# beecave-homelab/VibeVoice-ROCm

Measured on AMD Instinct MI355X. Metric: audio-sec/s, higher is better.
Workload: dtype bf16; 1 GPU; cfg2: VibeVoice-1.5B shapes, 1 speaker(s) x 203-frame voice prompt, 330-token prompt, 225 frames (30.0 s audio), CFG=2.0, 20 DPM-Solver++ steps, whole generate() incl. voice encode + prefill; global_batch=1, parallelism=replicas x1 (one dialogue per GPU), hipgraph=True

## Files before the change

vibevoice_rocm_amd/csrc/vv_common.h:

```cpp
#ifndef VV_COMMON_H
#define VV_COMMON_H
#include <hip/hip_runtime.h>
#include <stdarg.h>
#include <stdint.h>
#include "vv_hip.h"

int vv_set_error(int code, const char* fmt, ...);

#define VV_CHECK_LAUNCH(name)                                                                    \
  do {                                                                                           \
    hipError_t e_ = hipGetLastError();                                                           \
    if (e_ != hipSuccess) return vv_set_error(VV_E_HIP, "%s: %s", name, hipGetErrorString(e_));  \
  } while (0)

#define VV_TRY(expr)            \
  do {                          \
    int rc_ = (expr);           \
    if (rc_) return rc_;        \
  } while (0)

int vv_launch_gemv_stream(const vv_lin_args& a, hipStream_t s);
int vv_launch_gemv_rows(const vv_lin_args& a, float* part, size_t part_floats, int* tickets, size_t n_tickets, hipStream_t s);
size_t vv_gemv_rows_part_floats(int n, int dual);
size_t vv_gemv_rows_tickets(int n);
int vv_gemv_rows_init();
void vv_gemv_rows_set(int on, int blocks, int pers);
int vv_linear_ws(const vv_lin_args* a, const void* f1, const void* f2, float* part, size_t part_floats, int* tickets, size_t n_tickets,
                 vv_stream_t stream, const vv_w8* q1 = nullptr, const vv_w8* q2 = nullptr);
int vv_launch_mfma_gemm(const vv_lin_args& a, hipStream_t s);
int vv_mfma_gemm_init();
int vv_launch_attn_decode(const float* qkv, int64_t ld_qkv, int R, int heads, const vv_kv* kv, int layer, const float2* rope, const int* lens, float* out,
                          int64_t ldo, float* part, int* tickets, int nsplit, int part_cap, hipStream_t s);
int vv_attn_decode_ws(const float* qkv, int64_t ld_qkv, int R, int heads, const vv_kv* kv, int layer, const float* rope_table, const int* lens, float* out,
                      int64_t ldo, float* part, int* tickets, int nsplit, int part_cap, vv_stream_t stream);
int vv_launch_attn_prefill(const float* qkv, int64_t ld_qkv, int R, int heads, const vv_kv* kv, int layer, const int* lens, const int* cache_rows,
                           float* out, int64_t ldo, hipStream_t s);
int vv_head_init_fused(const vv_head* h, const float* noise, float* Xs, float* Ms, float* h0, int64_t ldh, hipStream_t s);
bool vv_head_boundary_supported(const vv_head* h);
int vv_head_boundary_fused(const vv_head* h, const float* hrows, int64_t ldh, const float* shift, const float* scale, int64_t ld_mod, float cfg,
                           const vv_dpm_coef* k, float* Xs, float* Ms, float* h_out, int64_t ldh_out, float* latent_out, hipStream_t s);
int vv_head_boundary_batch(const vv_head* h, const float* hrows, int64_t ldh, const float* shift, const float* scale, int64_t ld_mod, float cfg,
                           const vv_dpm_coef* k, float* Xs, float* Ms, int64_t state_stride, float* h_out, int64_t ldh_out, float* latent_out,
                           int64_t latent_stride, int B, hipStream_t s,
                           const float* nx = nullptr, int64_t nx_stride = 0);
int vv_head_sde_proj_fused(const vv_head* h, const float* sde_noise, int64_t ld_sde, int n_steps, int B, float* NX, hipStream_t s);
int vv_fused_init();
int vv_head_pre_fused(const vv_head* h, const float* cond2, int64_t ld_cond, const float* temb, int n_steps, void* c_bf16, const float* noise,
                      float* Xs, float* Ms, float* h0, int64_t ldh, hipStream_t s);
int vv_launch_connector_pair(const vv_connector* ac, const vv_connector* sem, const float* latent, const float* semfeat, float* out, int64_t ldo, int rows_out,
                             float* ws, hipStream_t s);
int vv_head_modulations_fused(const vv_head* h, const void* c_bf16, int rows, float* const* mod, float* modf, hipStream_t s);
struct vv_conv_ctx_item { float* pad; float* state; int ctx, T, C; const float* dw_w; float* hs; int affine; float scale, bias; };
int vv_conv_ctx_batch(const vv_conv_ctx_item* items, int n, int scatter, hipStream_t s);
int vv_block1d_init();
int vv_launch_block1d(const vv_block& B, int wdt, const float* x, float* out, int T, int C, float eps, hipStream_t s);
void vv_block1d_set_fused(int on);
void vv_block1d_set_blocks(int b);
int vv_convffn_init();
int vv_launch_convffn(const vv_block& B, int wdt, const float* x, float* y, void* hidden, float* hist_new, float* out, int T, int C, float eps,
                      hipStream_t s);
void vv_convffn_set(int on);
int vv_launch_ffn_in_row(const vv_block& B, int wdt, const float* x, float* y, float* hidden, float* hist_new, int C, float eps, hipStream_t s);
void vv_convffn_set_t1(int on);
int vv_launch_ffn_in_row_hs(const vv_block& B, int wdt, const float* x, float* y, float* hidden, float* hist_new, int C, float eps, hipStream_t s);
void vv_convffn_set_t1hs(int on);
void vv_convffn_set_rows(int c, int rows);
void vv_convffn_set_c128(int on);
bool vv_convffn_prefers(int wdt, int T, int C);
int vv_launch_skinny(const vv_lin_args& a, hipStream_t s);
void vv_skinny_set(int on, int min_m, int max_m);
int vv_rmsnorm_rows(const float* x, int64_t ldx, const float* w, float eps, int rows, int n, float* out, int64_t ldo, hipStream_t s);

#ifdef __HIPCC__
__device__ __forceinline__ float vv_gelu_as(float v) {
  const float x = v * 0.70710678118654752440f, ax = fabsf(x);
  const float t = __builtin_amdgcn_rcpf(fmaf(0.3275911f, ax, 1.0f));
  const float poly = t * fmaf(t, fmaf(t, fmaf(t, fmaf(t, 1.061405429f, -1.453152027f), 1.421413741f), -0.284496736f), 0.254829592f);
  const float erf_abs = 1.0f - poly * __expf(-ax * ax);
  return 0.5f * v * (1.0f + copysignf(erf_abs, x));
}

__device__ __forceinline__ float vv_wave_sum(float v) {
#define VV_DPP_ADD(ctrl) v += __int_as_float(__builtin_amdgcn_update_dpp(0, __float_as_int(v), ctrl, 0xF, 0xF, true))
  VV_DPP_ADD(0xB1);
  VV_DPP_ADD(0x4E);
  VV_DPP_ADD(0x141);
  VV_DPP_ADD(0x140);
#undef VV_DPP_ADD
  const float r0 = __int_as_float(__builtin_amdgcn_readlane(__float_as_int(v), 0));
  const float r1 = __int_as_float(__builtin_amdgcn_readlane(__float_as_int(v), 16));
  const float r2 = __int_as_float(__builtin_amdgcn_readlane(__float_as_int(v), 32));
  const float r3 = __int_as_float(__builtin_amdgcn_readlane(__float_as_int(v), 48));
  return (r0 + r1) + (r2 + r3);
}
#endif

#endif
```

vibevoice_rocm_amd/csrc/vv_convffn.hip:

```cpp
#include <hip/hip_runtime.h>
#include <hip/hip_bf16.h>
#include <stdint.h>

#include "vv_hip.h"
#include "vv_common.h"

namespace {

typedef unsigned short bf16_t;
typedef __bf16 bf16x8 __attribute__((ext_vector_type(8)));
typedef float f32x16 __attribute__((ext_vector_type(16)));
typedef float f32x4 __attribute__((ext_vector_type(4)));
typedef unsigned int u32x4 __attribute__((ext_vector_type(4)));

#ifdef VV_CF_TIMING
__device__ unsigned long long g_cf_t[8];
#define CSTAMP(i) do { if (blockIdx.x == 0 && blockIdx.y == 0 && threadIdx.x == 0) { const long long t_ = wall_clock64(); g_cf_t[i] += (unsigned long long)(t_ - tprev_); tprev_ = t_; } } while (0)
#else
#define CSTAMP(i) do { } while (0)
#endif

constexpr int TR2 = 16;
constexpr int HALO = 6;

__device__ __forceinline__ unsigned int pack2(float a, float b) {
  const __hip_bfloat16 x = __float2bfloat16(a), y = __float2bfloat16(b);
  return (unsigned int)(*reinterpret_cast<const bf16_t*>(&x)) | ((unsigned int)(*reinterpret_cast<const bf16_t*>(&y)) << 16);
}
__device__ __forceinline__ float sq4(const float4 v) { return v.x * v.x + v.y * v.y + v.z * v.z + v.w * v.w; }

template <int C, int TRV, int NT = 256> struct InLay {
  static constexpr int VW = C >= 256 ? 4 : 2;
  static constexpr int F4 = C / 4;
  static constexpr int FV = C / VW;
  static constexpr int TPR = FV < NT ? FV : NT;
  static constexpr int NWV = NT / 64;
  static constexpr int CPT = FV / TPR;
  static constexpr int RP = NT / TPR;
  static constexpr int NI = (TRV + HALO + RP - 1) / RP;
  static constexpr int WR = NI * RP;
  static constexpr int WPR = TPR / 64;
  static constexpr int P1 = C + 8;
  static constexpr int ST = C / (16 * NWV);
  static constexpr size_t XN = (size_t)WR * C * 4;
  static constexpr size_t RED = (size_t)NWV * 16 * 64 * 4;
  static constexpr size_t XH = (size_t)(WR - HALO) * P1 * 2;
  static constexpr size_t PART = (size_t)2 * WR * 8 * 4;
  static constexpr size_t LDS = (XN > RED ? XN : RED) + XH + PART;
};

template <int VW> __device__ __forceinline__ void ldv(const float* p, float (&o)[VW]) {
  if constexpr (VW == 4) { const float4 t = *reinterpret_cast<const float4*>(p); o[0] = t.x; o[1] = t.y; o[2] = t.z; o[3] = t.w; }
  else { const float2 t = *reinterpret_cast<const float2*>(p); o[0] = t.x; o[1] = t.y; }
}
template <int VW> __device__ __forceinline__ void stv(float* p, const float (&o)[VW]) {
  if constexpr (VW == 4) *reinterpret_cast<float4*>(p) = make_float4(o[0], o[1], o[2], o[3]);
  else *reinterpret_cast<float2*>(p) = make_float2(o[0], o[1]);
}

template <int C, int TRV, bool HF32, int NT>
__global__ __launch_bounds__(NT) void ffn_in_kernel(const float* __restrict__ x, float* __restrict__ y, void* __restrict__ hidden_v,
                                                     float* __restrict__ hist_new, int T, const vv_block B, float eps) {
  using L = InLay<C, TRV, NT>;
  constexpr int TR = TRV, CPT = L::CPT, VW = L::VW, NWV = L::NWV;
#ifdef VV_CF_TIMING
  long long tprev_ = wall_clock64();
#endif
  extern __shared__ __attribute__((aligned(16))) unsigned char smem[];
  float* xn = reinterpret_cast<float*>(smem);
  float* red = reinterpret_cast<float*>(smem);
  bf16_t* xh = reinterpret_cast<bf16_t*>(smem + (L::XN > L::RED ? L::XN : L::RED));
  float* part = reinterpret_cast<float*>(smem + (L::XN > L::RED ? L::XN : L::RED) + L::XH);
  float* part2 = part + L::WR * 8;
  const int tid = threadIdx.x, lane = tid & 63, wave = __builtin_amdgcn_readfirstlane(tid >> 6);
  const int n0 = blockIdx.x * 32;
  const int t0 = blockIdx.y * TR;
  const int rows = min(TR, T - t0);
  const int lm = lane & 31, hk = (lane >> 5) * 8;

  const int rloc = wave / L::WPR, slot = wave % L::WPR;
  int c0[CPT];
#pragma unroll
  for (int j = 0; j < CPT; ++j) c0[j] = VW * (tid % L::TPR + L::TPR * j);
  const float* hb = B.hist ? B.hist : x;
  const float hkeep = B.hist ? 1.f : 0.f;
  float own[L::NI][CPT][VW];
#pragma unroll
  for (int i = 0; i < L::NI; ++i) {
    const int w = rloc + L::RP * i, t = t0 - HALO + w;
    const bool isx = t >= 0;
    const float* src = isx ? x + (int64_t)min(t, T - 1) * C : hb + (int64_t)(B.hist ? HALO + t : 0) * C;
    const float keep = (w < rows + HALO) ? (isx ? 1.f : hkeep) : 0.f;
#pragma unroll
    for (int j = 0; j < CPT; ++j) {
      ldv<VW>(src + c0[j], own[i][j]);
#pragma unroll
      for (int e = 0; e < VW; ++e) own[i][j][e] *= keep;
    }
  }
  float nw[CPT][VW], db[CPT][VW], gm[CPT][VW], fw[CPT][VW];
  float tap[CPT][VW * 7];
#pragma unroll
  for (int j = 0; j < CPT; ++j) {
    ldv<VW>(B.norm_w + c0[j], nw[j]);
    ldv<VW>(B.dw_b + c0[j], db[j]);
    ldv<VW>(B.gamma + c0[j], gm[j]);
    ldv<VW>(B.ffn_norm_w + c0[j], fw[j]);
#pragma unroll
    for (int q = 0; q < 7; ++q) {
      float tq[VW];
      ldv<VW>(B.dw_w + (size_t)c0[j] * 7 + VW * q, tq);
#pragma unroll
      for (int e = 0; e < VW; ++e) tap[j][VW * q + e] = tq[e];
    }
  }
// ... 29 lines not shown
    for (int sl = 1; sl < L::WPR; ++sl) ss += part[w * 8 + sl];
    const bool isx = t >= 0;
    const float rstd = isx ? rsqrtf(ss / (float)C + eps) : 1.f;
#pragma unroll
    for (int j = 0; j < CPT; ++j) {
      float o[VW];
#pragma unroll
      for (int e = 0; e < VW; ++e) o[e] = own[i][j][e] * rstd * (isx ? nw[j][e] : 1.f);
      stv<VW>(xn + w * C + c0[j], o);
    }
  }
  __syncthreads();
  CSTAMP(2);

  float y1[L::NI][CPT][VW];
#pragma unroll
  for (int i = 0; i < L::NI; ++i) {
#pragma unroll
    for (int j = 0; j < CPT; ++j)
#pragma unroll
      for (int e = 0; e < VW; ++e) y1[i][j][e] = 0.f;
    if (L::RP * i + L::RP - 1 < HALO) continue;
    const int w = rloc + L::RP * i, tt = w - HALO;
    const int tc = max(tt, 0);
    const float ok = (tt >= 0 && tt < rows) ? 1.f : 0.f;
    float q = 0.f;
#pragma unroll
    for (int j = 0; j < CPT; ++j) {
      float s[VW];
#pragma unroll
      for (int e = 0; e < VW; ++e) s[e] = db[j][e];
#pragma unroll
      for (int k = 0; k < 7; ++k) {
        float v[VW];
        ldv<VW>(xn + (tc + k) * C + c0[j], v);
#pragma unroll
        for (int e = 0; e < VW; ++e) s[e] = fmaf(tap[j][7 * e + k], v[e], s[e]);
      }
#pragma unroll
      for (int e = 0; e < VW; ++e) {
        y1[i][j][e] = (own[i][j][e] + gm[j][e] * s[e]) * ok;
        q = fmaf(y1[i][j][e], y1[i][j][e], q);
      }
    }
    const float s2 = vv_wave_sum(q);
    if (lane == 0) part2[w * 8 + slot] = s2;
  }
  if (hist_new && blockIdx.x == 0 && t0 + TR >= T) {
    for (int e = tid; e < HALO * L::F4; e += NT) {
      const int j = e / L::F4, c4 = e - j * L::F4;
      *reinterpret_cast<float4*>(hist_new + (size_t)j * C + 4 * c4) = *reinterpret_cast<const float4*>(xn + (size_t)(T - t0 + j) * C + 4 * c4);
    }
  }
  __syncthreads();
  CSTAMP(3);
  {
    const int ys0 = blockIdx.x * (C / (int)gridDim.x);
#pragma unroll
    for (int i = 0; i < L::NI; ++i) {
      if (L::RP * i + L::RP - 1 < HALO) continue;
      const int w = rloc + L::RP * i, tt = w - HALO;
      if (tt >= 0) {
        float ss = part2[w * 8];
#pragma unroll
        for (int sl = 1; sl < L::WPR; ++sl) ss += part2[w * 8 + sl];
        const float rstd = rsqrtf(ss / (float)C + eps);
#pragma unroll
        for (int j = 0; j < CPT; ++j) {
          if constexpr (VW == 4) {
            uint2 p;
            p.x = pack2(y1[i][j][0] * rstd * fw[j][0], y1[i][j][1] * rstd * fw[j][1]);
            p.y = pack2(y1[i][j][2] * rstd * fw[j][2], y1[i][j][3] * rstd * fw[j][3]);
            *reinterpret_cast<uint2*>(xh + tt * L::P1 + c0[j]) = p;
          } else {
            *reinterpret_cast<unsigned int*>(xh + tt * L::P1 + c0[j]) = pack2(y1[i][j][0] * rstd * fw[j][0], y1[i][j][1] * rstd * fw[j][1]);
          }
          const bool mine = c0[j] >= ys0 && c0[j] < ys0 + C / (int)gridDim.x;
          if (mine && tt < rows) stv<VW>(y + (int64_t)(t0 + tt) * C + c0[j], y1[i][j]);
        }
      }
    }
  }
  __syncthreads();

  CSTAMP(4);
  f32x16 acc;
#pragma unroll
  for (int i = 0; i < 16; ++i) acc[i] = 0.f;
  {
    const bf16_t* xf = xh + min(lm, TR - 1) * L::P1 + wave * (C / NWV) + hk;
#pragma unroll
    for (int s = 0; s < L::ST; ++s) {
      const u32x4 xb = *reinterpret_cast<const u32x4*>(xf + s * 16);
      acc = __builtin_amdgcn_mfma_f32_32x32x16_bf16(__builtin_bit_cast(bf16x8, wf[s]), __builtin_bit_cast(bf16x8, xb), acc, 0, 0, 0);
    }
  }
#pragma unroll
  for (int r = 0; r < 16; ++r) red[(wave * 16 + r) * 64 + lane] = acc[r];
  __syncthreads();
  CSTAMP(5);
  {
    const int m = lane & 31;
    if (m < rows && wave < 4) {
      float v[4];
#pragma unroll
      for (int i = 0; i < 4; ++i) {
// ... 79 lines not shown
    }
  q2 = vv_wave_sum(q2);
  if (lane == 0) part[4 + wave] = q2;
  if (keeper) {
#pragma unroll
    for (int j = 0; j < 2; ++j) {
#pragma unroll
      for (int r = 0; r < 5; ++r) stv<4>(hist_new + (size_t)r * C + c0[j], hrow[r][j]);
      stv<4>(hist_new + (size_t)5 * C + c0[j], xn[j]);
    }
  }
  __syncthreads();
  const float rstd2 = rsqrtf(((part[4] + part[5]) + (part[6] + part[7])) / (float)C + eps);
  {
    const int ys0 = blockIdx.x * (C / (int)gridDim.x);
#pragma unroll
    for (int j = 0; j < 2; ++j) {
      uint2 p;
      p.x = pack2(yv[j][0] * rstd2 * fw[j][0], yv[j][1] * rstd2 * fw[j][1]);
      p.y = pack2(yv[j][2] * rstd2 * fw[j][2], yv[j][3] * rstd2 * fw[j][3]);
      *reinterpret_cast<uint2*>(xh + c0[j]) = p;
      if (c0[j] >= ys0 && c0[j] < ys0 + C / (int)gridDim.x) stv<4>(y + c0[j], yv[j]);
    }
  }
  __syncthreads();
  f32x16 acc;
#pragma unroll
  for (int i = 0; i < 16; ++i) acc[i] = 0.f;
  {
    const bf16_t* xf = xh + wave * (C / 4) + hk;
#pragma unroll
    for (int s = 0; s < ST; ++s) {
      const u32x4 xb = *reinterpret_cast<const u32x4*>(xf + s * 16);
      acc = __builtin_amdgcn_mfma_f32_32x32x16_bf16(__builtin_bit_cast(bf16x8, wf[s]), __builtin_bit_cast(bf16x8, xb), acc, 0, 0, 0);
    }
  }
#pragma unroll
  for (int r = 0; r < 16; ++r) red[(wave * 16 + r) * 64 + lane] = acc[r];
  __syncthreads();
  if ((lane & 31) == 0) {
    float v[4];
#pragma unroll
    for (int i = 0; i < 4; ++i) {
      float s = 0.f;
#pragma unroll
      for (int w4 = 0; w4 < 4; ++w4) s += red[(w4 * 16 + 4 * eg + i) * 64 + lane];
      v[i] = s;
    }
    *reinterpret_cast<float4*>(hidden + n0 + 8 * eg + 4 * (lane >> 5)) =
        make_float4(vv_gelu_as(v[0] + b1v.x), vv_gelu_as(v[1] + b1v.y), vv_gelu_as(v[2] + b1v.z), vv_gelu_as(v[3] + b1v.w));
  }
}

template <int C, int NW>
__global__ __launch_bounds__(64 * NW) void ffn_out_kernel(const bf16_t* __restrict__ hidden, const float* res, float* out, const float* __restrict__ hist_new,
                                                          int T, const vv_block B) {
  constexpr int K = 4 * C, KW = K / NW, ST = KW / 32;
  __shared__ float red[NW * 4 * 64];
  const int tid = threadIdx.x, lane = tid & 63, wave = tid >> 6;
  const int n0 = blockIdx.x * 16, t0 = blockIdx.y * TR2;
  const int r16 = lane & 15, kq = lane >> 4;
  u32x4 wf[ST], hf[ST];
  {
    const bf16_t* wr = reinterpret_cast<const bf16_t*>(B.w2) + (int64_t)(n0 + r16) * K + wave * KW + 8 * kq;
    const bf16_t* hr = hidden + (int64_t)min(t0 + r16, T - 1) * K + wave * KW + 8 * kq;
#pragma unroll
    for (int s = 0; s < ST; ++s) {
      wf[s] = *reinterpret_cast<const u32x4*>(wr + s * 32);
      hf[s] = *reinterpret_cast<const u32x4*>(hr + s * 32);
    }
  }
  const int ei = (tid >> 6) & 3, el = tid & 63;
  const int en = n0 + 4 * (el >> 4) + ei, em = t0 + (el & 15);
  const bool ev = em < T && tid < 256;
  const float b2v = B.b2[en], fgv = B.ffn_gamma[en];
  const float rv = ev ? res[(int64_t)em * C + en] : 0.f;
  const bool mover = hist_new && B.hist && blockIdx.x == 0 && blockIdx.y == 0;
  constexpr int HN = (HALO * C / 4 + 64 * NW - 1) / (64 * NW);
  float4 hv[HN];
  if (mover) {
#pragma unroll
    for (int i = 0; i < HN; ++i) {
      const int e = tid + 64 * NW * i;
      hv[i] = e < HALO * C / 4 ? *reinterpret_cast<const float4*>(hist_new + 4 * (size_t)e) : make_float4(0.f, 0.f, 0.f, 0.f);
    }
  }
  f32x4 acc = {0.f, 0.f, 0.f, 0.f};
#pragma unroll
  for (int s = 0; s < ST; ++s)
    acc = __builtin_amdgcn_mfma_f32_16x16x32_bf16(__builtin_bit_cast(bf16x8, wf[s]), __builtin_bit_cast(bf16x8, hf[s]), acc, 0, 0, 0);
#pragma unroll
  for (int i = 0; i < 4; ++i) red[(wave * 4 + i) * 64 + lane] = acc[i];
  __syncthreads();
  if (ev) {
    float s = 0.f;
#pragma unroll
    for (int w4 = 0; w4 < NW; ++w4) s += red[(w4 * 4 + ei) * 64 + el];
    out[(int64_t)em * C + en] = rv + fgv * (s + b2v);
  }
  if (mover) {
#pragma unroll
    for (int i = 0; i < HN; ++i) {
      const int e = tid + 64 * NW * i;
      if (e < HALO * C / 4) *reinterpret_cast<float4*>(B.hist + 4 * (size_t)e) = hv[i];
    }
  }
}

template <int NST, int NB>
__global__ __launch_bounds__(256) void skinny_kernel(const float* __restrict__ x, int64_t ldx, int M, const bf16_t* __restrict__ W, int K,
                                                     const float* __restrict__ bias, float* __restrict__ out, int64_t ldo) {
  __shared__ float red[4 * 4 * 64];
  const int tid = threadIdx.x, lane = tid & 63, wave = tid >> 6;
  const int n0 = blockIdx.x * 16, t0 = blockIdx.y * 16;
  const int r16 = lane & 15, kq = lane >> 4;
  const int kb = wave * (32 * NST * NB) + 8 * kq;
  const bf16_t* wr = W + (int64_t)(n0 + r16) * K + kb;
  const float* xr = x + (int64_t)min(t0 + r16, M - 1) * ldx + kb;
  const int ei = tid >> 6, el = tid & 63;
  const int en = n0 + 4 * (el >> 4) + ei, em = t0 + (el & 15);
  const float bv = bias ? bias[en] : 0.f;
  f32x4 acc = {0.f, 0.f, 0.f, 0.f};
#pragma unroll
  for (int b = 0; b < NB; ++b) {
    u32x4 wf[NST];
    float4 xa[NST], xb[NST];
#pragma unroll
    for (int s = 0; s < NST; ++s) {
      wf[s] = *reinterpret_cast<const u32x4*>(wr + 32 * (b * NST + s));
      xa[s] = *reinterpret_cast<const float4*>(xr + 32 * (b * NST + s));
      xb[s] = *reinterpret_cast<const float4*>(xr + 32 * (b * NST + s) + 4);
    }
#pragma unroll
    for (int s = 0; s < NST; ++s) {
      u32x4 p;
      p.x = pack2(xa[s].x, xa[s].y); p.y = pack2(xa[s].z, xa[s].w); p.z = pack2(xb[s].x, xb[s].y); p.w = pack2(xb[s].z, xb[s].w);
      acc = __builtin_amdgcn_mfma_f32_16x16x32_bf16(__builtin_bit_cast(bf16x8, wf[s]), __builtin_bit_cast(bf16x8, p), acc, 0, 0, 0);
    }
  }
#pragma unroll
  for (int i = 0; i < 4; ++i) red[(wave * 4 + i) * 64 + lane] = acc[i];
  __syncthreads();
  if (em < M) {
    float v = 0.f;
#pragma unroll
    for (int w4 = 0; w4 < 4; ++w4) v += red[(w4 * 4 + ei) * 64 + el];
    out[(int64_t)em * ldo + en] = v + bv;
  }
}

int g_skinny = 1, g_skinny_min_m = 5, g_skinny_max_m = 2048;

int g_on = 1;

template <int C> constexpr int in_threads() { return (C == 512 || C == 1024) ? 512 : 256; }

template <int C, int TRV, int NW>
int launch_c(const vv_block& B, const float* x, float* y, void* hidden, float* hist_new, float* out, int T, float eps, hipStream_t s) {
  float* hn = B.hist ? hist_new : nullptr;
  constexpr int NT = in_threads<C>();
  constexpr size_t lds = InLay<C, TRV, NT>::LDS;
  hipLaunchKernelGGL((ffn_in_kernel<C, TRV, false, NT>), dim3(4 * C / 32, (T + TRV - 1) / TRV), dim3(NT), lds, s, x, y, hidden, hn, T, B, eps);
  hipLaunchKernelGGL((ffn_out_kernel<C, NW>), dim3(C / 16, (T + TR2 - 1) / TR2), dim3(64 * NW), 0, s, reinterpret_cast<const bf16_t*>(hidden), y, out, hn, T, B);
  return hipGetLastError() == hipSuccess ? 1 : vv_set_error(VV_E_HIP, "vv_convffn: launch failed");
}

int g_trv512 = 8, g_trv256 = 16, g_trv128 = 32;
int g_c128 = 1;

}

#ifdef VV_CF_TIMING
extern "C" int vv_convffn_debug_times(unsigned long long* out8, int reset) {
  if (hipMemcpyFromSymbol(out8, HIP_SYMBOL(g_cf_t), 8 * sizeof(unsigned long long)) != hipSuccess) return -1;
  if (reset) { unsigned long long z[8] = {0}; if (hipMemcpyToSymbol(HIP_SYMBOL(g_cf_t), z, sizeof(z)) != hipSuccess) return -1; }
  return 0;
}
#endif
void vv_convffn_set(int on) { g_on = on; }
void vv_convffn_set_rows(int c, int rows) { if (c == 512) g_trv512 = rows; else if (c == 256) g_trv256 = rows; else if (c == 128) g_trv128 = rows; }
void vv_convffn_set_c128(int on) { g_c128 = on; }
bool vv_convffn_prefers(int wdt, int T, int C) { return g_on && g_c128 && wdt == VV_BF16 && C == 128 && T >= 3 && T <= 1024; }
void vv_skinny_set(int on, int min_m, int max_m) { g_skinny = on; if (min_m > 0) g_skinny_min_m = min_m; if (max_m > 0) g_skinny_max_m = max_m; }

int vv_launch_skinny(const vv_lin_args& a, hipStream_t s) {
  if (!g_skinny || a.wdt != VV_BF16 || a.w2 || a.pro != VV_PRO_NONE || a.act != VV_ACT_NONE || a.gate || a.res || a.mod_scale || a.flags) return 0;
  if (a.m < g_skinny_min_m || a.m > g_skinny_max_m || a.n % 16 || a.ldx % 4 || a.ldx == 0 || ((uintptr_t)a.x % 16) || ((uintptr_t)a.w % 16)) return 0;
  dim3 grid(a.n / 16, (a.m + 15) / 16);
  const bf16_t* W = reinterpret_cast<const bf16_t*>(a.w);
#define VV_SK(NSTV, NBV) hipLaunchKernelGGL((skinny_kernel<NSTV, NBV>), grid, dim3(256), 0, s, a.x, a.ldx, a.m, W, a.k, a.bias, a.out, a.ldo)
  switch (a.k) {
    case 128: VV_SK(1, 1); break;
    case 256: VV_SK(2, 1); break;
    case 512: VV_SK(4, 1); break;
    case 1024: VV_SK(8, 1); break;
    case 2048: VV_SK(16, 1); break;
    case 2560: VV_SK(20, 1); break;
    case 5120: VV_SK(20, 2); break;
    default: return 0;
  }
#undef VV_SK
  return 1;
}

int vv_convffn_init() {
#define VV_CF_ATTR(CC, TT)                                                                                                                  \
  { constexpr int nt_ = in_threads<CC>(); constexpr int l_ = (int)InLay<CC, TT, nt_>::LDS;                                                 \
    if (hipFuncSetAttribute(reinterpret_cast<const void*>(&ffn_in_kernel<CC, TT, false, nt_>), hipFuncAttributeMaxDynamicSharedMemorySize, l_) != hipSuccess) \
      return vv_set_error(VV_E_HIP, "vv_convffn_init: cannot raise the LDS limit"); }
  VV_CF_ATTR(128, 16) VV_CF_ATTR(128, 32) VV_CF_ATTR(256, 8) VV_CF_ATTR(256, 16) VV_CF_ATTR(256, 32) VV_CF_ATTR(512, 8) VV_CF_ATTR(512, 16) VV_CF_ATTR(512, 32) VV_CF_ATTR(1024, 8)
#undef VV_CF_ATTR
  {
    constexpr int l1 = (int)InLay<2048, 1, 256>::LDS;
    if (hipFuncSetAttribute(reinterpret_cast<const void*>(&ffn_in_kernel<2048, 1, true, 256>), hipFuncAttributeMaxDynamicSharedMemorySize, l1) != hipSuccess)
      return vv_set_error(VV_E_HIP, "vv_convffn_init: cannot raise the LDS limit");
  }
  return 0;
}

int g_t1 = 1;
void vv_convffn_set_t1(int on) { g_t1 = on; }

int vv_launch_ffn_in_row(const vv_block& B, int wdt, const float* x, float* y, float* hidden, float* hist_new, int C, float eps, hipStream_t s) {
  if (!g_on || !g_t1 || wdt != VV_BF16 || C != 2048 || !B.hist) return 0;
  auto a16 = [](const void* q) { return q && ((uintptr_t)q % 16) == 0; };
  if (!a16(B.w1) || !a16(B.b1) || !a16(B.gamma) || !a16(B.norm_w) || !a16(B.ffn_norm_w) || !a16(B.dw_b) || !a16(B.dw_w) || !a16(x) || !a16(y) ||
      !a16(hidden) || !a16(hist_new) || !a16(B.hist) || x == y)
    return 0;
  constexpr size_t lds = InLay<2048, 1, 256>::LDS;
  hipLaunchKernelGGL((ffn_in_kernel<2048, 1, true, 256>), dim3(4 * 2048 / 32, 1), dim3(256), lds, s, x, y, hidden, hist_new, 1, B, eps);
  return hipGetLastError() == hipSuccess ? 1 : vv_set_error(VV_E_HIP, "vv_convffn: launch failed");
}

int g_t1hs = 1;
void vv_convffn_set_t1hs(int on) { g_t1hs = on; }

int vv_launch_ffn_in_row_hs(const vv_block& B, int wdt, const float* x, float* y, float* hidden, float* hist_new, int C, float eps, hipStream_t s) {
  if (!g_on || !g_t1 || !g_t1hs || wdt != VV_BF16 || C != 2048 || !B.hist || !B.hs || !B.dw_last) return 0;
  auto a16 = [](const void* q) { return q && ((uintptr_t)q % 16) == 0; };
  if (!a16(B.w1) || !a16(B.b1) || !a16(B.gamma) || !a16(B.norm_w) || !a16(B.ffn_norm_w) || !a16(B.dw_b) || !a16(B.dw_last) || !a16(B.hs) || !a16(x) ||
      !a16(y) || !a16(hidden) || !a16(hist_new) || !a16(B.hist) || x == y)
    return 0;
  hipLaunchKernelGGL(ffn_in_row_kernel, dim3(4 * 2048 / 32), dim3(256), 0, s, x, y, hidden, hist_new, B, eps);
  return hipGetLastError() == hipSuccess ? 1 : vv_set_error(VV_E_HIP, "vv_convffn: launch failed");
}

int vv_launch_convffn(const vv_block& B, int wdt, const float* x, float* y, void* hidden, float* hist_new, float* out, int T, int C, float eps,
                      hipStream_t s) {
  if (!g_on || wdt != VV_BF16 || T < 3 || (C != 128 && C != 256 && C != 512 && C != 1024) || (C == 1024 && T > 64)) return 0;
  if (C == 128 ? (!g_c128 || T > 1024) : T > 256) return 0;
  auto a16 = [](const void* q) { return q && ((uintptr_t)q % 16) == 0; };
  if (!a16(B.w1) || !a16(B.w2) || !a16(B.b1) || !B.b2 || !a16(B.gamma) || !B.ffn_gamma || !a16(B.norm_w) || !a16(B.ffn_norm_w) || !a16(B.dw_b) ||
      !a16(B.dw_w) || !a16(x) || !a16(y) || !a16(hidden) || !a16(hist_new) || !out || (B.hist && !a16(B.hist)))
    return 0;
  {
    const uintptr_t xa = (uintptr_t)x, ya = (uintptr_t)y, bytes = (uintptr_t)T * C * 4;
    if (xa < ya + bytes && ya < xa + bytes) return 0;
  }
  if (C == 128) {
    if (g_trv128 == 16) return launch_c<128, 16, 4>(B, x, y, hidden, hist_new, out, T, eps, s);
    return launch_c<128, 32, 4>(B, x, y, hidden, hist_new, out, T, eps, s);
  }
  if (C == 256) {
    if (g_trv256 == 8) return launch_c<256, 8, 4>(B, x, y, hidden, hist_new, out, T, eps, s);
    if (g_trv256 == 16) return launch_c<256, 16, 4>(B, x, y, hidden, hist_new, out, T, eps, s);
    return launch_c<256, 32, 4>(B, x, y, hidden, hist_new, out, T, eps, s);
  }
  if (C == 512) {
    if (g_trv512 == 8) return launch_c<512, 8, 4>(B, x, y, hidden, hist_new, out, T, eps, s);
    if (g_trv512 == 16) return launch_c<512, 16, 4>(B, x, y, hidden, hist_new, out, T, eps, s);
    return launch_c<512, 32, 4>(B, x, y, hidden, hist_new, out, T, eps, s);
  }
  return launch_c<1024, 8, 8>(B, x, y, hidden, hist_new, out, T, eps, s);
}

extern "C" size_t vv_block_mid_ws_bytes(int T, int C) { return (size_t)T * C * 4 + (size_t)T * 4 * C * 2 + (size_t)HALO * C * 4 + 64; }

extern "C" int vv_block_mid(const vv_block* b, int wdt, const float* x, float* out, void* ws, int T, int C, float eps, vv_stream_t stream) {
  if (!b || !x || !out || !ws || T <= 0) return vv_set_error(VV_E_ARG, "vv_block_mid: bad args");
  float* y = reinterpret_cast<float*>(ws);
  char* hidden = reinterpret_cast<char*>(ws) + (size_t)T * C * 4;
  float* hn = reinterpret_cast<float*>(hidden + (size_t)T * 4 * C * 2);
  const int rc = vv_launch_convffn(*b, wdt, x, y, hidden, hn, out, T, C, eps, (hipStream_t)stream);
  if (rc < 0) return rc;
  if (rc == 0) return vv_set_error(VV_E_UNSUPPORTED, "vv_block_mid: shape not covered (C=%d T=%d wdt=%d)", C, T, wdt);
  return 0;
}
```

vibevoice_rocm_amd/csrc/vv_kernels.hip:

```cpp
#include <hip/hip_runtime.h>
#include <hip/hip_bf16.h>
#include <stdint.h>
#include <stdio.h>
#include <string.h>
#include <math.h>

#include "vv_hip.h"
#include "vv_common.h"

static thread_local char g_err[512] = "";

int vv_set_error(int code, const char* fmt, ...) {
  va_list ap;
  va_start(ap, fmt);
  vsnprintf(g_err, sizeof(g_err), fmt, ap);
  va_end(ap);
  return code;
}

extern "C" const char* vv_last_error(void) { return g_err; }
extern "C" int vv_abi_version(void) { return 6; }
int vv_mixer_init();
extern "C" int vv_init(void) {
  VV_TRY(vv_mixer_init());
// ... 9 lines not shown
static int rows_scratch(int on) {
  if (on && !g_rows_part) {
    if (hipMalloc(&g_rows_part, G_ROWS_PART_FLOATS * sizeof(float)) != hipSuccess || hipMalloc(&g_rows_tk, G_ROWS_TICKETS * sizeof(int)) != hipSuccess ||
        hipMemset(g_rows_tk, 0, G_ROWS_TICKETS * sizeof(int)) != hipSuccess)
      return vv_set_error(VV_E_HIP, "vv_tune: gemv_rows_scratch allocation failed");
  }
  if (!on && g_rows_part) { (void)hipFree(g_rows_part); (void)hipFree(g_rows_tk); g_rows_part = nullptr; g_rows_tk = nullptr; }
  return 0;
}
void vv_gemv_rows_set_dbg(int d);
void vv_gemv_rows_set_atomic(int on);
void vv_gemv_stream_set_blocks(int b);
void vv_gemv_stream_set_waves(int w);
void vv_gemv_stream_set_opt(int o);
void vv_gemv_stream_set_long(int cap, int ku);
void vv_gemv_stream_set_dual_rw(int r);
void vv_gemv_stream_set_small_rw(int r);
void vv_mfma_set_mt(int mt);
void vv_mfma_set_tiled_rows(int r);
void vv_mfma_set_tiled_bk128(int on);
void vv_mfma_set_tiled_small(int t);
void vv_mfma_set_tiled_dual_bk64(int on);
void vv_mfma_set_tiled_small_dual(int t);
void vv_mfma_set_tiled_small_k(int k);
void vv_mixer_set_rows(int on);
void vv_mfma_set_mt_prefill(int mt);
extern int g_attn_group;
void vv_attn_decode_set_gqa(int on);
void vv_attn_decode_set_gqa_keys(int k);
extern "C" int vv_tune(const char* key, int value) {
  if (key && !strcmp(key, "gemv_long_cap")) { vv_gemv_stream_set_long(value, 0); return 0; }
  if (key && !strcmp(key, "gemv_long_ku")) { vv_gemv_stream_set_long(0, value); return 0; }
  if (key && !strcmp(key, "gemv_blocks")) { vv_gemv_stream_set_blocks(value); return 0; }
  if (key && !strcmp(key, "gemv_waves")) { vv_gemv_stream_set_waves(value); return 0; }
  if (key && !strcmp(key, "gemv_rows")) { vv_gemv_rows_set(value, 0, -1); return 0; }
  if (key && !strcmp(key, "gemv_rows_blocks")) { vv_gemv_rows_set(-1, value, -1); return 0; }
  if (key && !strcmp(key, "gemv_rows_pers")) { vv_gemv_rows_set(-1, 0, value); return 0; }
  if (key && !strcmp(key, "gemv_rows_scratch")) return rows_scratch(value);
  if (key && !strcmp(key, "gemv_rows_dbg")) { vv_gemv_rows_set_dbg(value); return 0; }
  if (key && !strcmp(key, "gemv_rows_atomic")) { vv_gemv_rows_set_atomic(value); return 0; }
  if (key && !strcmp(key, "gemv_opt")) { vv_gemv_stream_set_opt(value); return 0; }
  if (key && !strcmp(key, "gemv_dual_rw")) { vv_gemv_stream_set_dual_rw(value); return 0; }
  if (key && !strcmp(key, "gemv_small_rw")) { vv_gemv_stream_set_small_rw(value); return 0; }
  if (key && !strcmp(key, "mixer_rows")) { vv_mixer_set_rows(value); return 0; }
  if (key && !strcmp(key, "block1d_fused")) { vv_block1d_set_fused(value); return 0; }
  if (key && !strcmp(key, "block1d_blocks")) { vv_block1d_set_blocks(value); return 0; }
  if (key && !strcmp(key, "convffn")) { vv_convffn_set(value); return 0; }
  if (key && !strcmp(key, "convffn_t1")) { vv_convffn_set_t1(value); return 0; }
  if (key && !strcmp(key, "convffn_t1hs")) { vv_convffn_set_t1hs(value); return 0; }
  if (key && !strcmp(key, "convffn_rows512")) { vv_convffn_set_rows(512, value); return 0; }
  if (key && !strcmp(key, "convffn_rows256")) { vv_convffn_set_rows(256, value); return 0; }
  if (key && !strcmp(key, "convffn_rows128")) { vv_convffn_set_rows(128, value); return 0; }
  if (key && !strcmp(key, "convffn_c128")) { vv_convffn_set_c128(value); return 0; }
  if (key && !strcmp(key, "skinny")) { vv_skinny_set(value, 0, 0); return 0; }
  if (key && !strcmp(key, "skinny_min_m")) { vv_skinny_set(1, value, 0); return 0; }
  if (key && !strcmp(key, "skinny_max_m")) { vv_skinny_set(1, 0, value); return 0; }
  if (key && !strcmp(key, "mfma_tiled_bk128")) { vv_mfma_set_tiled_bk128(value); return 0; }
  if (key && !strcmp(key, "attn_group")) { g_attn_group = value; return 0; }
  if (key && !strcmp(key, "attn_gqa")) { vv_attn_decode_set_gqa(value); return 0; }
  if (key && !strcmp(key, "attn_gqa_keys")) { vv_attn_decode_set_gqa_keys(value); return 0; }
  if (key && !strcmp(key, "mfma_tiled_small_k")) { vv_mfma_set_tiled_small_k(value); return 0; }
  if (key && !strcmp(key, "mfma_tiled_dual_bk64")) { vv_mfma_set_tiled_dual_bk64(value); return 0; }
  if (key && !strcmp(key, "mfma_tiled_small_dual")) { vv_mfma_set_tiled_small_dual(value); return 0; }
  if (key && !strcmp(key, "mfma_tiled_small")) { vv_mfma_set_tiled_small(value); return 0; }
  if (key && !strcmp(key, "mfma_tiled_rows")) { vv_mfma_set_tiled_rows(value); return 0; }
  if (key && !strcmp(key, "mfma_mt")) { vv_mfma_set_mt(value); return 0; }
  if (key && !strcmp(key, "mfma_mt_prefill")) { vv_mfma_set_mt_prefill(value); return 0; }
  return vv_set_error(VV_E_ARG, "vv_tune: unknown key");
}

typedef unsigned short bf16_t;

__device__ __forceinline__ float bf2f(unsigned int u16) { return __uint_as_float(u16 << 16); }
__device__ __forceinline__ float wave_sum(float v) {
#pragma unroll
  for (int o = 32; o > 0; o >>= 1) v += __shfl_xor(v, o);
  return v;
}
__device__ __forceinline__ float wave_sum_dpp(float v) { return vv_wave_sum(v); }
__device__ __forceinline__ float silu_f(float v) { return v / (1.0f + expf(-v)); }
__device__ __forceinline__ float gelu_f(float v) { return 0.5f * v * (1.0f + erff(v * 0.70710678118654752440f)); }

template <typename WT> struct WL;
template <> struct WL<float> {
  static __device__ __forceinline__ void load8(const float* p, float (&o)[8]) {
    const float4 a = *reinterpret_cast<const float4*>(p);
    const float4 b = *reinterpret_cast<const float4*>(p + 4);
    o[0] = a.x; o[1] = a.y; o[2] = a.z; o[3] = a.w; o[4] = b.x; o[5] = b.y; o[6] = b.z; o[7] = b.w;
  }
  static __device__ __forceinline__ void load4(const float* p, float (&o)[4]) {
    const float4 a = *reinterpret_cast<const float4*>(p);
    o[0] = a.x; o[1] = a.y; o[2] = a.z; o[3] = a.w;
  }
  static __device__ __forceinline__ float load1(const float* p) { return *p; }
};
template <> struct WL<bf16_t> {
  static __device__ __forceinline__ void load8(const bf16_t* p, float (&o)[8]) {
    const uint4 v = *reinterpret_cast<const uint4*>(p);
    o[0] = __uint_as_float(v.x << 16); o[1] = __uint_as_float(v.x & 0xffff0000u);
    o[2] = __uint_as_float(v.y << 16); o[3] = __uint_as_float(v.y & 0xffff0000u);
    o[4] = __uint_as_float(v.z << 16); o[5] = __uint_as_float(v.z & 0xffff0000u);
    o[6] = __uint_as_float(v.w << 16); o[7] = __uint_as_float(v.w & 0xffff0000u);
  }
  static __device__ __forceinline__ void load4(const bf16_t* p, float (&o)[4]) {
    const uint2 v = *reinterpret_cast<const uint2*>(p);
    o[0] = __uint_as_float(v.x << 16); o[1] = __uint_as_float(v.x & 0xffff0000u);
// ... 1567 lines not shown
```

vibevoice_rocm_amd/csrc/vv_model.hip:

```cpp
#include <hip/hip_runtime.h>
#include <stdint.h>
#include <string.h>

#include "vv_hip.h"
#include "vv_common.h"

namespace {

struct Carver {
  char* p;
  explicit Carver(void* base) : p(reinterpret_cast<char*>(base)) {}
  float* take(size_t n_floats) {
    float* r = reinterpret_cast<float*>(p);
    p += (n_floats * sizeof(float) + 255) & ~(size_t)255;
    return r;
  }
};
inline size_t al(size_t n_floats) { return (n_floats * sizeof(float) + 255) & ~(size_t)255; }

inline vv_lin_args lin_base(const float* x, int64_t ldx, int m, const void* w, int n, int k, int wdt, float* out, int64_t ldo) {
  vv_lin_args a;
  memset(&a, 0, sizeof(a));
  a.x = x; a.ldx = ldx; a.m = m; a.w = w; a.n = n; a.k = k; a.wdt = wdt; a.out = out; a.ldo = ldo;
  return a;
// ... 363 lines not shown
  VV_TRY(head_modulations(h, c, (int)R, mod, modf, true, true, stream));
  for (int b = 0; b < B; ++b)
    VV_TRY(vv_head_init_fused(h, noise + (size_t)b * ld_noise, Xs + (size_t)b * sst, Ms + (size_t)b * sst, hb[0] + (size_t)2 * b * D, D, s));
  for (int i = 0; i < n_steps; ++i) {
    float* hc = hb[i & 1];
    for (int l = 0; l < h->layers; ++l) {
      const vv_head_layer& L = h->layer[l];
      const float* ml = mod[l] + (size_t)R2 * i * 3 * D;
      a = lin_base(hc, D, R2, L.wgate, h->ffn, D, h->wdt, act, h->ffn);
      a.pro = VV_PRO_RMSNORM; a.norm_w = L.norm_w; a.eps = h->eps;
      a.mod_shift = ml; a.mod_scale = ml + D; a.ld_mod = 3 * D;
      a.w2 = L.wup; a.act = VV_ACT_SWIGLU; a.flags = VV_LIN_W_REUSED;
      VV_TRY(vv_linear_ws(&a, L.f_gate, L.f_up, rpart, rpart_n, rtick, rtick_n, stream, f8q ? &L.q_gate : nullptr, f8q ? &L.q_up : nullptr));
      a = lin_base(act, h->ffn, R2, L.wdown, D, h->ffn, h->wdt, hc, D);
      a.gate = ml + 2 * D; a.gate_ld = 3 * D; a.res = hc; a.ldres = D; a.flags = VV_LIN_W_REUSED;
      VV_TRY(vv_linear_ws(&a, L.f_down, nullptr, rpart, rpart_n, rtick, rtick_n, stream, f8q ? &L.q_down : nullptr));
    }
    const float* mf = modf + (size_t)R2 * i * 2 * D;
    VV_TRY(vv_head_boundary_batch(h, hc, D, mf, mf + D, 2 * D, cfg_scale, &coef[i], Xs, Ms, sst, hb[(i + 1) & 1], D, latent_out, ld_latent, B, s,
                                  NX ? NX + (size_t)i * sst : nullptr, (int64_t)n_steps * sst));
  }
  return 0;
}

extern "C" int vv_head_sample_batch(const vv_head* h, const float* cond, int64_t ld_cond, const float* noise, int64_t ld_noise, const float* temb,
                                    const vv_dpm_coef* coef, int n_steps, float cfg_scale, float* latent_out, int64_t ld_latent, int B, void* ws,
                                    vv_stream_t stream) {
  return head_sample_batch(nullptr, h, cond, ld_cond, noise, ld_noise, temb, coef, n_steps, cfg_scale, latent_out, ld_latent, B, ws,
                           nullptr, 0, stream);
}

extern "C" int vv_head_sample_batch_sde(const vv_head* h, const float* cond, int64_t ld_cond, const float* noise, int64_t ld_noise, const float* temb,
                                        const vv_dpm_coef* coef, int n_steps, float cfg_scale, float* latent_out, int64_t ld_latent, int B, void* ws,
                                        const float* sde_noise, int64_t ld_sde, vv_stream_t stream) {
  return head_sample_batch("vv_head_sample_batch_sde", h, cond, ld_cond, noise, ld_noise, temb, coef, n_steps, cfg_scale, latent_out, ld_latent, B, ws,
                           sde_noise, ld_sde, stream);
}

static inline int conv_ctx_of(const vv_conv& c) { return c.transposed ? 1 : c.kk - c.stride; }

static void convnet_sizes(const vv_convnet* net, int64_t t_in, int decoder, size_t* act_elems, size_t* hid_elems) {
  size_t amax = 0, hmax = 0;
  int64_t T = t_in;
  for (int i = 0; i < net->n_stages; ++i) {
    const vv_conv& cv = net->sample[i];
    const int ctx = conv_ctx_of(cv);
    size_t in_el = (size_t)(T + ctx + cv.kk + cv.stride) * cv.cin;
    if (in_el > amax) amax = in_el;
    if (cv.transposed) T = T * cv.stride; else T = (T + cv.stride - 1) / cv.stride;
    const size_t C = cv.cout;
    size_t el = (size_t)(T + 8) * C;
    if (el > amax) amax = el;
    if (net->n_blocks[i] > 0 && (size_t)T * 4 * C > hmax) hmax = (size_t)T * 4 * C;
  }
  size_t in_el = (size_t)(T + 8 + net->head.kk) * net->head.cin;
  if (in_el > amax) amax = in_el;
  (void)decoder;
  *act_elems = amax + 64;
  *hid_elems = hmax + 64;
}

static bool convnet_streaming(const vv_convnet* net) {
  for (int i = 0; i <= net->n_stages; ++i) {
    const vv_conv& cv = (i == net->n_stages) ? net->head : net->sample[i];
    if (conv_ctx_of(cv) > 0 && !cv.state) return false;
  }
  return true;
}
static size_t convnet_pad_floats(const vv_convnet* net, int64_t t_in, size_t* offs ) {
  size_t tot = 0;
  int64_t T = t_in;
  for (int i = 0; i <= net->n_stages; ++i) {
    const vv_conv& cv = (i == net->n_stages) ? net->head : net->sample[i];
    if (offs) offs[i] = tot;
    tot += (((size_t)(T + conv_ctx_of(cv) + 2) * cv.cin) + 63) & ~(size_t)63;
    if (cv.transposed) T = T * cv.stride; else T = (T + cv.stride - 1) / cv.stride;
  }
  return tot;
}

#define VV_ROW_BLOCKS 16
#define VV_ROW_HIST_FLOATS ((size_t)VV_ROW_BLOCKS * 6 * 2048)
#define VV_CTX_ITEMS (VV_MAX_STAGES + 1 + 16)

extern "C" size_t vv_convnet_ws_bytes(const vv_convnet* net, int64_t t_in, int decoder) {
  if (!net || t_in <= 0) return 0;
  VV_WQ_STRIP(vv_convnet, net);
  size_t a, h;
  convnet_sizes(net, t_in, decoder, &a, &h);
  return 2 * al(a) + al(h) + (convnet_streaming(net) ? al(convnet_pad_floats(net, t_in, nullptr)) + al(VV_ROW_HIST_FLOATS) : 0);
}

static int run_blocks(const vv_convnet* net, int wq, int stage, int64_t T, int C, float*& cur, float*& other, float* hid,
                      int nctx, float** pad_out, vv_stream_t stream, float* next_pad = nullptr, float* row_hist = nullptr,
                      vv_conv_ctx_item* items = nullptr, int* n_items = nullptr, int* row_stage = nullptr) {
  const int nb = net->n_blocks[stage];
  for (int j = 0; j < nb; ++j) {
    const vv_block& B = net->blocks[stage][j];
    const bool last = (j == nb - 1);
    if (!vv_convffn_prefers(net->wdt, (int)T, C)) {
      float* dst = last ? (next_pad ? next_pad : other) + (size_t)nctx * C : other;
      const int fused = vv_launch_block1d(B, net->wdt, cur, dst, (int)T, C, net->eps, (hipStream_t)stream);
      if (fused < 0) return fused;
      if (fused) {
        if (last) { *pad_out = next_pad ? next_pad : other; cur = nullptr; }
        else { float* t = cur; cur = other; other = t; }
// ... 305 lines not shown
```

Measured before the change: 38.39 audio-sec/s.

## Split-K the conv FFN output GEMM with ticketed last-block reduction

Adds a K-split (KSP=4) to the ffn_out_kernel for C=512 and C=1024. Each split writes its partial sums to a scratch buffer and bumps a per-tile ticket, and the last arriving block reduces the partials and writes the output. Tickets are zeroed by the preceding ffn_in_kernel. The aim is more blocks and parallelism for the small-T acoustic decoder/encoder FFN, in exchange for extra scratch memory, atomics, and a serialized final reduction; C=1024 also drops from 8 to 4 waves per block.

```diff
diff --git a/vibevoice_rocm_amd/csrc/vv_common.h b/vibevoice_rocm_amd/csrc/vv_common.h
--- a/vibevoice_rocm_amd/csrc/vv_common.h
+++ b/vibevoice_rocm_amd/csrc/vv_common.h
@@ -67,6 +67,8 @@
 void vv_convffn_set_rows(int c, int rows);
 void vv_convffn_set_c128(int on);
 bool vv_convffn_prefers(int wdt, int T, int C);
+void vv_convffn_set_ksp(int c, int ksp);
+size_t vv_convffn_scratch_floats(int T, int C);
 int vv_launch_skinny(const vv_lin_args& a, hipStream_t s);
 void vv_skinny_set(int on, int min_m, int max_m);
 int vv_rmsnorm_rows(const float* x, int64_t ldx, const float* w, float eps, int rows, int n, float* out, int64_t ldo, hipStream_t s);
diff --git a/vibevoice_rocm_amd/csrc/vv_convffn.hip b/vibevoice_rocm_amd/csrc/vv_convffn.hip
--- a/vibevoice_rocm_amd/csrc/vv_convffn.hip
+++ b/vibevoice_rocm_amd/csrc/vv_convffn.hip
@@ -60,7 +60,8 @@
 
 template <int C, int TRV, bool HF32, int NT>
 __global__ __launch_bounds__(NT) void ffn_in_kernel(const float* __restrict__ x, float* __restrict__ y, void* __restrict__ hidden_v,
-                                                     float* __restrict__ hist_new, int T, const vv_block B, float eps) {
+                                                     float* __restrict__ hist_new, int* __restrict__ tickets, int n_tickets, int T,
+                                                     const vv_block B, float eps) {
   using L = InLay<C, TRV, NT>;
   constexpr int TR = TRV, CPT = L::CPT, VW = L::VW, NWV = L::NWV;
 #ifdef VV_CF_TIMING
@@ -196,6 +197,8 @@
       *reinterpret_cast<float4*>(hist_new + (size_t)j * C + 4 * c4) = *reinterpret_cast<const float4*>(xn + (size_t)(T - t0 + j) * C + 4 * c4);
     }
   }
+  if (blockIdx.x == 0 && blockIdx.y == 0)
+    for (int e = tid; e < n_tickets; e += NT) tickets[e] = 0;
   __syncthreads();
   CSTAMP(3);
   {
@@ -381,18 +384,20 @@
   }
 }
 
-template <int C, int NW>
+template <int C, int NW, int KSP>
 __global__ __launch_bounds__(64 * NW) void ffn_out_kernel(const bf16_t* __restrict__ hidden, const float* res, float* out, const float* __restrict__ hist_new,
-                                                          int T, const vv_block B) {
-  constexpr int K = 4 * C, KW = K / NW, ST = KW / 32;
+                                                          float* part, int* tickets, int T, const vv_block B) {
+  constexpr int K = 4 * C, KW = K / (NW * KSP), ST = KW / 32;
   __shared__ float red[NW * 4 * 64];
+  __shared__ int s_last;
   const int tid = threadIdx.x, lane = tid & 63, wave = tid >> 6;
-  const int n0 = blockIdx.x * 16, t0 = blockIdx.y * TR2;
+  const int n0 = blockIdx.x * 16, t0 = blockIdx.y * TR2, ks = KSP > 1 ? (int)blockIdx.z : 0;
   const int r16 = lane & 15, kq = lane >> 4;
   u32x4 wf[ST], hf[ST];
   {
-    const bf16_t* wr = reinterpret_cast<const bf16_t*>(B.w2) + (int64_t)(n0 + r16) * K + wave * KW + 8 * kq;
-    const bf16_t* hr = hidden + (int64_t)min(t0 + r16, T - 1) * K + wave * KW + 8 * kq;
+    const int kb = ks * (K / KSP) + wave * KW + 8 * kq;
+    const bf16_t* wr = reinterpret_cast<const bf16_t*>(B.w2) + (int64_t)(n0 + r16) * K + kb;
+    const bf16_t* hr = hidden + (int64_t)min(t0 + r16, T - 1) * K + kb;
 #pragma unroll
     for (int s = 0; s < ST; ++s) {
       wf[s] = *reinterpret_cast<const u32x4*>(wr + s * 32);
@@ -404,7 +409,7 @@
   const bool ev = em < T && tid < 256;
   const float b2v = B.b2[en], fgv = B.ffn_gamma[en];
   const float rv = ev ? res[(int64_t)em * C + en] : 0.f;
-  const bool mover = hist_new && B.hist && blockIdx.x == 0 && blockIdx.y == 0;
+  const bool mover = hist_new && B.hist && blockIdx.x == 0 && blockIdx.y == 0 && ks == 0;
   constexpr int HN = (HALO * C / 4 + 64 * NW - 1) / (64 * NW);
   float4 hv[HN];
   if (mover) {
@@ -421,12 +426,6 @@
 #pragma unroll
   for (int i = 0; i < 4; ++i) red[(wave * 4 + i) * 64 + lane] = acc[i];
   __syncthreads();
-  if (ev) {
-    float s = 0.f;
-#pragma unroll
-    for (int w4 = 0; w4 < NW; ++w4) s += red[(w4 * 4 + ei) * 64 + el];
-    out[(int64_t)em * C + en] = rv + fgv * (s + b2v);
-  }
   if (mover) {
 #pragma unroll
     for (int i = 0; i < HN; ++i) {
@@ -434,6 +433,31 @@
       if (e < HALO * C / 4) *reinterpret_cast<float4*>(B.hist + 4 * (size_t)e) = hv[i];
     }
   }
+  float s = 0.f;
+  if (tid < 256) {
+#pragma unroll
+    for (int w4 = 0; w4 < NW; ++w4) s += red[(w4 * 4 + ei) * 64 + el];
+  }
+  if constexpr (KSP > 1) {
+    const int tile = blockIdx.y * gridDim.x + blockIdx.x;
+    float* pp = part + (int64_t)tile * KSP * 256;
+    if (tid < 256) __hip_atomic_store(pp + ks * 256 + tid, s, __ATOMIC_RELAXED, __HIP_MEMORY_SCOPE_AGENT);
+    asm volatile("s_waitcnt vmcnt(0)" ::: "memory");
+    __syncthreads();
+    if (tid == 0) {
+      const int tk = __hip_atomic_fetch_add(&tickets[tile], 1, __ATOMIC_RELAXED, __HIP_MEMORY_SCOPE_AGENT);
+      s_last = (tk == KSP - 1);
+    }
+    __syncthreads();
+    if (!s_last || tid >= 256) return;
+    float pv[KSP];
+#pragma unroll
+    for (int i = 0; i < KSP; ++i) pv[i] = __hip_atomic_load(pp + i * 256 + tid, __ATOMIC_RELAXED, __HIP_MEMORY_SCOPE_AGENT);
+    s = pv[0];
+#pragma unroll
+    for (int i = 1; i < KSP; ++i) s += pv[i];
+  }
+  if (ev) out[(int64_t)em * C + en] = rv + fgv * (s + b2v);
 }
 
 template <int NST, int NB>
@@ -484,18 +508,28 @@
 
 template <int C> constexpr int in_threads() { return (C == 512 || C == 1024) ? 512 : 256; }
 
-template <int C, int TRV, int NW>
-int launch_c(const vv_block& B, const float* x, float* y, void* hidden, float* hist_new, float* out, int T, float eps, hipStream_t s) {
-  float* hn = B.hist ? hist_new : nullptr;
+constexpr int KSP_MAX = 4;
+__host__ __device__ constexpr int out_tiles(int T, int C) { return (C / 16) * ((T + TR2 - 1) / TR2); }
+constexpr size_t part_off(int C) { return (size_t)HALO * C; }
+constexpr size_t tick_off(int T, int C) { return part_off(C) + (size_t)out_tiles(T, C) * KSP_MAX * 256; }
+
+template <int C, int TRV, int NW, int KSP>
+int launch_c(const vv_block& B, const float* x, float* y, void* hidden, float* scratch, float* out, int T, float eps, hipStream_t s) {
+  float* hn = B.hist ? scratch : nullptr;
+  float* part = scratch + part_off(C);
+  int* tickets = reinterpret_cast<int*>(scratch + tick_off(T, C));
+  const int nt = KSP > 1 ? out_tiles(T, C) : 0;
   constexpr int NT = in_threads<C>();
   constexpr size_t lds = InLay<C, TRV, NT>::LDS;
-  hipLaunchKernelGGL((ffn_in_kernel<C, TRV, false, NT>), dim3(4 * C / 32, (T + TRV - 1) / TRV), dim3(NT), lds, s, x, y, hidden, hn, T, B, eps);
-  hipLaunchKernelGGL((ffn_out_kernel<C, NW>), dim3(C / 16, (T + TR2 - 1) / TR2), dim3(64 * NW), 0, s, reinterpret_cast<const bf16_t*>(hidden), y, out, hn, T, B);
+  hipLaunchKernelGGL((ffn_in_kernel<C, TRV, false, NT>), dim3(4 * C / 32, (T + TRV - 1) / TRV), dim3(NT), lds, s, x, y, hidden, hn, tickets, nt, T, B, eps);
+  hipLaunchKernelGGL((ffn_out_kernel<C, NW, KSP>), dim3(C / 16, (T + TR2 - 1) / TR2, KSP), dim3(64 * NW), 0, s, reinterpret_cast<const bf16_t*>(hidden), y, out, hn,
+                     part, tickets, T, B);
   return hipGetLastError() == hipSuccess ? 1 : vv_set_error(VV_E_HIP, "vv_convffn: launch failed");
 }
 
 int g_trv512 = 8, g_trv256 = 16, g_trv128 = 32;
 int g_c128 = 1;
+int g_ksp1024 = 4, g_ksp512 = 4;
 
 }
 
@@ -509,6 +543,10 @@
 void vv_convffn_set(int on) { g_on = on; }
 void vv_convffn_set_rows(int c, int rows) { if (c == 512) g_trv512 = rows; else if (c == 256) g_trv256 = rows; else if (c == 128) g_trv128 = rows; }
 void vv_convffn_set_c128(int on) { g_c128 = on; }
+void vv_convffn_set_ksp(int c, int ksp) {
+  if (c == 1024) g_ksp1024 = ksp; else if (c == 512) g_ksp512 = ksp;
+}
+size_t vv_convffn_scratch_floats(int T, int C) { return tick_off(T, C) + (size_t)out_tiles(T, C) + 16; }
 bool vv_convffn_prefers(int wdt, int T, int C) { return g_on && g_c128 && wdt == VV_BF16 && C == 128 && T >= 3 && T <= 1024; }
 void vv_skinny_set(int on, int min_m, int max_m) { g_skinny = on; if (min_m > 0) g_skinny_min_m = min_m; if (max_m > 0) g_skinny_max_m = max_m; }
 
@@ -557,7 +595,7 @@
       !a16(hidden) || !a16(hist_new) || !a16(B.hist) || x == y)
     return 0;
   constexpr size_t lds = InLay<2048, 1, 256>::LDS;
-  hipLaunchKernelGGL((ffn_in_kernel<2048, 1, true, 256>), dim3(4 * 2048 / 32, 1), dim3(256), lds, s, x, y, hidden, hist_new, 1, B, eps);
+  hipLaunchKernelGGL((ffn_in_kernel<2048, 1, true, 256>), dim3(4 * 2048 / 32, 1), dim3(256), lds, s, x, y, hidden, hist_new, nullptr, 0, 1, B, eps);
   return hipGetLastError() == hipSuccess ? 1 : vv_set_error(VV_E_HIP, "vv_convffn: launch failed");
 }
 
@@ -587,23 +625,25 @@
     if (xa < ya + bytes && ya < xa + bytes) return 0;
   }
   if (C == 128) {
-    if (g_trv128 == 16) return launch_c<128, 16, 4>(B, x, y, hidden, hist_new, out, T, eps, s);
-    return launch_c<128, 32, 4>(B, x, y, hidden, hist_new, out, T, eps, s);
+    if (g_trv128 == 16) return launch_c<128, 16, 4, 1>(B, x, y, hidden, hist_new, out, T, eps, s);
+    return launch_c<128, 32, 4, 1>(B, x, y, hidden, hist_new, out, T, eps, s);
   }
   if (C == 256) {
-    if (g_trv256 == 8) return launch_c<256, 8, 4>(B, x, y, hidden, hist_new, out, T, eps, s);
-    if (g_trv256 == 16) return launch_c<256, 16, 4>(B, x, y, hidden, hist_new, out, T, eps, s);
-    return launch_c<256, 32, 4>(B, x, y, hidden, hist_new, out, T, eps, s);
+    if (g_trv256 == 8) return launch_c<256, 8, 4, 1>(B, x, y, hidden, hist_new, out, T, eps, s);
+    if (g_trv256 == 16) return launch_c<256, 16, 4, 1>(B, x, y, hidden, hist_new, out, T, eps, s);
+    return launch_c<256, 32, 4, 1>(B, x, y, hidden, hist_new, out, T, eps, s);
   }
   if (C == 512) {
-    if (g_trv512 == 8) return launch_c<512, 8, 4>(B, x, y, hidden, hist_new, out, T, eps, s);
-    if (g_trv512 == 16) return launch_c<512, 16, 4>(B, x, y, hidden, hist_new, out, T, eps, s);
-    return launch_c<512, 32, 4>(B, x, y, hidden, hist_new, out, T, eps, s);
-  }
-  return launch_c<1024, 8, 8>(B, x, y, hidden, hist_new, out, T, eps, s);
-}
-
-extern "C" size_t vv_block_mid_ws_bytes(int T, int C) { return (size_t)T * C * 4 + (size_t)T * 4 * C * 2 + (size_t)HALO * C * 4 + 64; }
+    if (g_ksp512 == 4 && g_trv512 == 8) return launch_c<512, 8, 4, 4>(B, x, y, hidden, hist_new, out, T, eps, s);
+    if (g_trv512 == 8) return launch_c<512, 8, 4, 1>(B, x, y, hidden, hist_new, out, T, eps, s);
+    if (g_trv512 == 16) return launch_c<512, 16, 4, 1>(B, x, y, hidden, hist_new, out, T, eps, s);
+    return launch_c<512, 32, 4, 1>(B, x, y, hidden, hist_new, out, T, eps, s);
+  }
+  if (g_ksp1024 == 4) return launch_c<1024, 8, 4, 4>(B, x, y, hidden, hist_new, out, T, eps, s);
+  return launch_c<1024, 8, 8, 1>(B, x, y, hidden, hist_new, out, T, eps, s);
+}
+
+extern "C" size_t vv_block_mid_ws_bytes(int T, int C) { return (size_t)T * C * 4 + (size_t)T * 4 * C * 2 + vv_convffn_scratch_floats(T, C) * 4 + 64; }
 
 extern "C" int vv_block_mid(const vv_block* b, int wdt, const float* x, float* out, void* ws, int T, int C, float eps, vv_stream_t stream) {
   if (!b || !x || !out || !ws || T <= 0) return vv_set_error(VV_E_ARG, "vv_block_mid: bad args");
diff --git a/vibevoice_rocm_amd/csrc/vv_kernels.hip b/vibevoice_rocm_amd/csrc/vv_kernels.hip
--- a/vibevoice_rocm_amd/csrc/vv_kernels.hip
+++ b/vibevoice_rocm_amd/csrc/vv_kernels.hip
@@ -85,6 +85,8 @@
   if (key && !strcmp(key, "convffn_rows256")) { vv_convffn_set_rows(256, value); return 0; }
   if (key && !strcmp(key, "convffn_rows128")) { vv_convffn_set_rows(128, value); return 0; }
   if (key && !strcmp(key, "convffn_c128")) { vv_convffn_set_c128(value); return 0; }
+  if (key && !strcmp(key, "convffn_ksp1024")) { vv_convffn_set_ksp(1024, value); return 0; }
+  if (key && !strcmp(key, "convffn_ksp512")) { vv_convffn_set_ksp(512, value); return 0; }
   if (key && !strcmp(key, "skinny")) { vv_skinny_set(value, 0, 0); return 0; }
   if (key && !strcmp(key, "skinny_min_m")) { vv_skinny_set(1, value, 0); return 0; }
   if (key && !strcmp(key, "skinny_max_m")) { vv_skinny_set(1, 0, value); return 0; }
diff --git a/vibevoice_rocm_amd/csrc/vv_model.hip b/vibevoice_rocm_amd/csrc/vv_model.hip
--- a/vibevoice_rocm_amd/csrc/vv_model.hip
+++ b/vibevoice_rocm_amd/csrc/vv_model.hip
@@ -439,6 +439,8 @@
     size_t el = (size_t)(T + 8) * C;
     if (el > amax) amax = el;
     if (net->n_blocks[i] > 0 && (size_t)T * 4 * C > hmax) hmax = (size_t)T * 4 * C;
+    if (net->n_blocks[i] > 0 && (size_t)T * 2 * C + vv_convffn_scratch_floats((int)T, (int)C) > hmax)
+      hmax = (size_t)T * 2 * C + vv_convffn_scratch_floats((int)T, (int)C);
   }
   size_t in_el = (size_t)(T + 8 + net->head.kk) * net->head.cin;
   if (in_el > amax) amax = in_el;
```

After: 38.64 audio-sec/s, median of 6. About the same (+0.7%).
